# pySTEPS/pysteps

Measured on NVIDIA H100. Metric: Mpix/s advected (2048^2 frame, 12 leadtimes), higher is better.
Workload: dtype f64 (trajectories, motion field, IDW); f32 precip in/out; u8/i16/f32 OpenCV-exact LK stages

## Files before the change

### pysteps_b200/csrc/lk_track.cu

```cuda
#include "common.cuh"

namespace {

constexpr int LK_MAX_LEVELS = 8;
constexpr int LK_THREADS = 128;
constexpr int W_BITS = 14;

struct LKParams {
    const uint8_t *I, *J;
    const short2 *dI;
    size_t off[LK_MAX_LEVELS];
    int h[LK_MAX_LEVELS], w[LK_MAX_LEVELS];
    int max_level;
    int win_w, win_h, max_count;
    double eps2, min_eig_thr;
    const float *prev_pts;
    const int *npts_dev;
    int npts;
    float *next_pts;
    uint8_t *status;
};

__device__ __forceinline__ int reflect101(int i, int L) {
    if (L == 1) return 0;
    while (i < 0 || i >= L) {
        if (i < 0) i = -i;
        if (i >= L) i = 2 * L - 2 - i;
    }
    return i;
}

__device__ __forceinline__ int descale(int x, int n) { return (x + (1 << (n - 1))) >> n; }

__device__ __forceinline__ int div_small(int i, float inv_d) { return __float2int_rd(((float)i + 0.5f) * inv_d); }

__device__ __forceinline__ void make_weights(float a, float b, int &w00, int &w01, int &w10, int &w11) {
    w00 = __float2int_rn((1.f - a) * (1.f - b) * (float)(1 << W_BITS));
    w01 = __float2int_rn(a * (1.f - b) * (float)(1 << W_BITS));
    w10 = __float2int_rn((1.f - a) * b * (float)(1 << W_BITS));
    w11 = (1 << W_BITS) - w00 - w01 - w10;
}

__global__ void __launch_bounds__(LK_THREADS) lk_track_kernel(const LKParams p) {
    extern __shared__ __align__(16) unsigned char smem_raw[];
    const int npts = p.npts_dev ? min(*p.npts_dev, p.npts) : p.npts;
    const int pt = blockIdx.x;
    if (pt >= npts) return;
    const int tid = threadIdx.x;
    const int ww = p.win_w, wh = p.win_h, npx = ww * wh;
    const int simd_w = (ww / 8) * 8;
    const int nchunk = simd_w / 8, ntail = ww - simd_w;
    short *Iw = (short *)smem_raw;
    short *Dx = Iw + npx;
    short *Dy = Dx + npx;
    const int npair = wh * nchunk * 4, ntl = wh * ntail;
    float *PX = (float *)(Dy + npx + (npx & 1));
    float *PY = PX + npair;
    float *TXp = PY + npair;
    float *TYp = TXp + ntl;
    float *red = TYp + ntl;
    __shared__ float s_b[2];

    const float inv_ww = 1.0f / (float)ww, inv_nchunk = nchunk > 0 ? 1.0f / (float)nchunk : 0.f,
                inv_ntail = ntail > 0 ? 1.0f / (float)ntail : 0.f;
    const float half_x = (ww - 1) * 0.5f, half_y = (wh - 1) * 0.5f;
    const float FLT_SCALE = 1.f / (float)(1 << 20);
    const int ct = tid - 32 * (blockIdx.x & (LK_THREADS / 32 - 1));
    float nx_out = 0.f, ny_out = 0.f;
    bool status = true;

    for (int level = p.max_level; level >= 0; level--) {
        const uint8_t *I = p.I + p.off[level];
        const uint8_t *J = p.J + p.off[level];
        const short2 *dI = p.dI + p.off[level];
        const int h = p.h[level], w = p.w[level];
        const float inv = (float)(1. / (double)(1 << level));
        float px = p.prev_pts[2 * pt] * inv, py = p.prev_pts[2 * pt + 1] * inv;
        float nx, ny;
        if (level == p.max_level) { nx = px; ny = py; }
        else { nx = nx_out * 2.f; ny = ny_out * 2.f; }
        nx_out = nx; ny_out = ny;
        px -= half_x; py -= half_y;
        const int ix = __float2int_rd(px), iy = __float2int_rd(py);
        if (ix < -ww || ix >= w || iy < -wh || iy >= h) {
            if (level == 0) status = false;
            continue;
        }
        int w00, w01, w10, w11;
        make_weights(px - (float)ix, py - (float)iy, w00, w01, w10, w11);

        __syncthreads();
        const bool inI = ix >= 0 && iy >= 0 && ix + ww < w && iy + wh < h;
        for (int i = tid; i < npx; i += LK_THREADS) {
            const int y = div_small(i, inv_ww), x = i - y * ww;
            const int yy = iy + y, xx = ix + x;
            int v00, v01, v10, v11;
            short2 d00 = make_short2(0, 0), d01 = d00, d10 = d00, d11 = d00;
            if (inI) {
                const uint8_t *q0 = I + (size_t)yy * w + xx;
                v00 = q0[0]; v01 = q0[1]; v10 = q0[w]; v11 = q0[w + 1];
                const short2 *g0 = dI + (size_t)yy * w + xx;
                d00 = g0[0]; d01 = g0[1]; d10 = g0[w]; d11 = g0[w + 1];
            } else {
                const int r0 = reflect101(yy, h), r1 = reflect101(yy + 1, h);
                const int c0 = reflect101(xx, w), c1 = reflect101(xx + 1, w);
                v00 = I[(size_t)r0 * w + c0]; v01 = I[(size_t)r0 * w + c1];
                v10 = I[(size_t)r1 * w + c0]; v11 = I[(size_t)r1 * w + c1];
                const bool y0in = yy >= 0 && yy < h, y1in = yy + 1 >= 0 && yy + 1 < h;
                const bool x0in = xx >= 0 && xx < w, x1in = xx + 1 >= 0 && xx + 1 < w;
                if (y0in && x0in) d00 = dI[(size_t)yy * w + xx];
                if (y0in && x1in) d01 = dI[(size_t)yy * w + xx + 1];
                if (y1in && x0in) d10 = dI[(size_t)(yy + 1) * w + xx];
                if (y1in && x1in) d11 = dI[(size_t)(yy + 1) * w + xx + 1];
            }
            Iw[i] = (short)descale(v00 * w00 + v01 * w01 + v10 * w10 + v11 * w11, W_BITS - 5);
            Dx[i] = (short)descale(d00.x * w00 + d01.x * w01 + d10.x * w10 + d11.x * w11, W_BITS);
            Dy[i] = (short)descale(d00.y * w00 + d01.y * w01 + d10.y * w10 + d11.y * w11, W_BITS);
        }
        __syncthreads();

        if (ct >= 0 && ct < 15) {
            const int acc = ct < 12 ? ct >> 2 : ct - 12;
            const short *pa = acc == 2 ? Dy : Dx, *pb = acc == 0 ? Dx : Dy;
            float q = 0.f;
            if (ct < 12) {
                const int l = ct & 3;
                for (int y = 0; y < wh; y++) {
                    const short *ra = pa + y * ww, *rb = pb + y * ww;
#pragma unroll 4
                    for (int x = l; x < simd_w; x += 4) q = __fmul_rn((float)ra[x], (float)rb[x]) + q;
                }
            } else {
                for (int y = 0; y < wh; y++)
                    for (int x = simd_w; x < ww; x++) q += (float)((int)pa[y * ww + x] * (int)pb[y * ww + x]);
            }
            red[ct] = q;
        }
        __syncthreads();
        float A[3];
#pragma unroll
        for (int a = 0; a < 3; a++) {
            const float s = (red[4 * a + 0] + red[4 * a + 2]) + (red[4 * a + 1] + red[4 * a + 3]);
            A[a] = (red[12 + a] + s) * FLT_SCALE;
        }
        const float A11 = A[0], A12 = A[1], A22 = A[2];
        float D = A11 * A22 - A12 * A12;
        const float minEig = (A22 + A11 - sqrtf((A11 - A22) * (A11 - A22) + 4.f * A12 * A12)) /
                             (float)(2 * ww * wh);
        if ((double)minEig < p.min_eig_thr || D < 1.1920928955078125e-07f) {
            if (level == 0) status = false;
            continue;
        }
        D = 1.f / D;
        nx -= half_x; ny -= half_y;
        float pdx = 0.f, pdy = 0.f;
        for (int j = 0; j < p.max_count; j++) {
            const int jx = __float2int_rd(nx), jy = __float2int_rd(ny);
            if (jx < -ww || jx >= w || jy < -wh || jy >= h) {
                if (level == 0) status = false;
                break;
            }
            make_weights(nx - (float)jx, ny - (float)jy, w00, w01, w10, w11);
            __syncthreads();
            const bool inJ = jx >= 0 && jy >= 0 && jx + ww < w && jy + wh < h;
            auto mismatch = [&](int y, int x) -> int {
                int v00, v01, v10, v11;
                if (inJ) {
                    const uint8_t *q0 = J + (size_t)(jy + y) * w + (jx + x);
                    v00 = q0[0]; v01 = q0[1]; v10 = q0[w]; v11 = q0[w + 1];
                } else {
                    const int r0 = reflect101(jy + y, h), r1 = reflect101(jy + y + 1, h);
                    const int c0 = reflect101(jx + x, w), c1 = reflect101(jx + x + 1, w);
                    v00 = J[(size_t)r0 * w + c0]; v01 = J[(size_t)r0 * w + c1];
                    v10 = J[(size_t)r1 * w + c0]; v11 = J[(size_t)r1 * w + c1];
                }
                const int jv = descale(v00 * w00 + v01 * w01 + v10 * w10 + v11 * w11, W_BITS - 5);
                return jv - (int)Iw[y * ww + x];
            };
            for (int i = tid; i < npair; i += LK_THREADS) {
                const int q = i & 3, y = div_small(i >> 2, inv_nchunk), c = (i >> 2) - y * nchunk;
                const int x0 = 8 * c + q, i0 = y * ww + x0;
                const int d0 = mismatch(y, x0), d1 = mismatch(y, x0 + 4);
                PX[i] = (float)(d0 * (int)Dx[i0] + d1 * (int)Dx[i0 + 4]);
                PY[i] = (float)(d0 * (int)Dy[i0] + d1 * (int)Dy[i0 + 4]);
            }
            for (int i = tid; i < ntl; i += LK_THREADS) {
                const int y = div_small(i, inv_ntail), x = simd_w + (i - y * ntail);
                const int d0 = mismatch(y, x);
                TXp[i] = (float)(d0 * (int)Dx[y * ww + x]);
                TYp[i] = (float)(d0 * (int)Dy[y * ww + x]);
            }
            __syncthreads();
            if (ct >= 0 && ct < 10) {
                float q = 0.f;
                if (ct < 8) {
                    const int pair = (ct >> 2) * 2 + ((ct & 3) >> 1);
                    const float *P = (ct & 1) ? PY : PX;
                    const int nsteps = wh * nchunk;
#pragma unroll 8
                    for (int s = 0; s < nsteps; s++) q += P[4 * s + pair];
                } else {
                    const float *P = (ct == 9) ? TYp : TXp;
#pragma unroll 4
                    for (int s = 0; s < ntl; s++) q += P[s];
                }
                red[ct] = q;
            }
            __syncthreads();
            if (ct == 0) {
                const float X0 = red[0] + red[4], Y0 = red[1] + red[5];
                const float X1 = red[2] + red[6], Y1 = red[3] + red[7];
                s_b[0] = (red[8] + ((X0 + 0.f) + (X1 + 0.f))) * FLT_SCALE;
                s_b[1] = (red[9] + ((Y0 + 0.f) + (Y1 + 0.f))) * FLT_SCALE;
            }
            __syncthreads();
            const float b1 = s_b[0], b2 = s_b[1];
            const float ddx = (A12 * b2 - A22 * b1) * D;
            const float ddy = (A12 * b1 - A11 * b2) * D;
            nx += ddx; ny += ddy;
            nx_out = nx + half_x; ny_out = ny + half_y;
            if ((double)ddx * (double)ddx + (double)ddy * (double)ddy <= p.eps2) break;
            if (j > 0 && fabs((double)(ddx + pdx)) < 0.01 && fabs((double)(ddy + pdy)) < 0.01) {
                nx_out -= ddx * 0.5f; ny_out -= ddy * 0.5f;
                break;
            }
            pdx = ddx; pdy = ddy;
        }
        if (status && level == 0) {
            const int fx = __float2int_rd(nx_out - half_x), fy = __float2int_rd(ny_out - half_y);
            if (fx < -ww || fx >= w || fy < -wh || fy >= h) status = false;
        }
    }
    if (tid == 0) {
        p.next_pts[2 * pt] = nx_out;
        p.next_pts[2 * pt + 1] = ny_out;
        p.status[pt] = status ? 1 : 0;
    }
}

__global__ void __launch_bounds__(1024)
compact_tracks_kernel(const float *__restrict__ p0, const float *__restrict__ p1,
                      const uint8_t *__restrict__ st, const int *__restrict__ npts_dev, int npts_cap,
                      double *__restrict__ pool_xy, double *__restrict__ pool_uv, int *__restrict__ pool_count,
                      int pool_cap) {
    __shared__ int warp_tot[32];
    __shared__ int s_base;
    const int npts = npts_dev ? min(*npts_dev, npts_cap) : npts_cap;
    const int tid = threadIdx.x, lane = tid & 31, wid = tid >> 5;
    if (tid == 0) s_base = *pool_count;
    __syncthreads();
    for (int start = 0; start < npts; start += blockDim.x) {
        const int i = start + tid;
        const bool keep = i < npts && st[i] == 1;
        const unsigned bal = __ballot_sync(0xffffffffu, keep);
        if (lane == 0) warp_tot[wid] = __popc(bal);
        __syncthreads();
        int before = 0, total = 0;
        for (int k = 0; k < (int)(blockDim.x >> 5); k++) {
            if (k < wid) before += warp_tot[k];
            total += warp_tot[k];
        }
        if (keep) {
            const int o = s_base + before + __popc(bal & ((1u << lane) - 1u));
            if (o < pool_cap) {
                const float x0 = p0[2 * i], y0 = p0[2 * i + 1];
                pool_xy[2 * o] = (double)x0;
                pool_xy[2 * o + 1] = (double)y0;
                pool_uv[2 * o] = (double)(p1[2 * i] - x0);
                pool_uv[2 * o + 1] = (double)(p1[2 * i + 1] - y0);
            }
        }
        __syncthreads();
        if (tid == 0) s_base = min(s_base + total, pool_cap);
        __syncthreads();
    }
    if (tid == 0) *pool_count = s_base;
}

}

extern "C" int b200_lk_pyramid_layout(int h, int w, int win_w, int win_h, int max_level,
                                      int *levels_out, int64_t *offsets , int *hs, int *ws,
                                      int64_t *total_pixels) {
    B200_REQUIRE(h >= 1 && w >= 1 && win_w >= 1 && win_h >= 1 && max_level >= 0, "bad arguments");
    if (max_level > LK_MAX_LEVELS - 1) max_level = LK_MAX_LEVELS - 1;
    int lv = 0;
    int64_t off = 0;
    int ch = h, cw = w;
    for (int level = 0;; level++) {
        if (offsets) offsets[level] = off;
        if (hs) hs[level] = ch;
        if (ws) ws[level] = cw;
        off += (int64_t)ch * cw;
        lv = level;
        if (level == max_level) break;
        const int nh = (ch + 1) / 2, nw = (cw + 1) / 2;
        if (nw <= win_w || nh <= win_h) break;
        ch = nh; cw = nw;
    }
    if (levels_out) *levels_out = lv;
    if (total_pixels) *total_pixels = off;
    return 0;
}

extern "C" int b200_pyr_down_u8(const uint8_t *src, int h, int w, uint8_t *dst, void *stream);
extern "C" int b200_scharr_i16(const uint8_t *src, int h, int w, int16_t *dst, void *stream);

extern "C" int b200_lk_build_pyramid(const uint8_t *img, int h, int w, int win_w, int win_h,
                                     int max_level, uint8_t *pyr, int16_t *deriv, void *stream) {
    B200_REQUIRE(pyr && (img || deriv), "bad arguments");
    int lv, hs[LK_MAX_LEVELS], ws[LK_MAX_LEVELS];
    int64_t off[LK_MAX_LEVELS], total;
    int rc = b200_lk_pyramid_layout(h, w, win_w, win_h, max_level, &lv, off, hs, ws, &total);
    if (rc) return rc;
    cudaStream_t s = (cudaStream_t)stream;
    if (img) {
        B200_CUDA(cudaMemcpyAsync(pyr, img, (size_t)h * w, cudaMemcpyDeviceToDevice, s));
        for (int l = 1; l <= lv; l++) {
            rc = b200_pyr_down_u8(pyr + off[l - 1], hs[l - 1], ws[l - 1], pyr + off[l], stream);
            if (rc) return rc;
        }
    }
    if (deriv)
        for (int l = 0; l <= lv; l++) {
            rc = b200_scharr_i16(pyr + off[l], hs[l], ws[l], deriv + 2 * off[l], stream);
            if (rc) return rc;
        }
    return 0;
}

extern "C" int b200_lk_track(const uint8_t *pyrI, const uint8_t *pyrJ, const int16_t *derivI, int h,
                             int w, int win_w, int win_h, int max_level, int max_count, double epsilon,
                             double min_eig_thr, const float *prev_pts, int npts, const int *npts_dev,
                             float *next_pts, uint8_t *status, void *stream) {
    B200_REQUIRE(pyrI && pyrJ && derivI && prev_pts && next_pts && status, "bad arguments");
    B200_REQUIRE(win_w >= 1 && win_h >= 1 && win_w * win_h <= 64 * 64, "window must be 1..64x64 pixels");
    if (npts <= 0) return 0;
    LKParams p;
    memset(&p, 0, sizeof(p));
    int lv;
    int64_t off[LK_MAX_LEVELS], total;
    int rc = b200_lk_pyramid_layout(h, w, win_w, win_h, max_level, &lv, off, p.h, p.w, &total);
    if (rc) return rc;
    for (int l = 0; l <= lv; l++) p.off[l] = (size_t)off[l];
    p.I = pyrI; p.J = pyrJ; p.dI = (const short2 *)derivI;
    p.max_level = lv;
    p.win_w = win_w; p.win_h = win_h;
    p.max_count = max_count;
    p.eps2 = epsilon * epsilon;
    p.min_eig_thr = min_eig_thr;
    p.prev_pts = prev_pts;
    p.npts = npts; p.npts_dev = npts_dev;
    p.next_pts = next_pts; p.status = status;
    const int npx = win_w * win_h;
    const int nchunk = win_w / 8, ntail = win_w - nchunk * 8;
    const size_t smem = sizeof(short) * (3 * (size_t)npx + (npx & 1)) +
                        sizeof(float) * (2 * (size_t)win_h * nchunk * 4 + 2 * (size_t)win_h * ntail + 16);
    B200_CUDA(cudaFuncSetAttribute(lk_track_kernel, cudaFuncAttributeMaxDynamicSharedMemorySize, (int)smem));
    lk_track_kernel<<<npts, LK_THREADS, smem, (cudaStream_t)stream>>>(p);
    B200_LAUNCH_CHECK();
    return 0;
}

extern "C" int b200_lk_compact_tracks(const float *p0, const float *p1, const uint8_t *status,
                                      const int *npts_dev, int npts_cap, double *pool_xy,
                                      double *pool_uv, int *pool_count, int pool_cap, void *stream) {
    B200_REQUIRE(p0 && p1 && status && pool_xy && pool_uv && pool_count && npts_cap >= 0 && pool_cap >= 0,
                 "bad arguments");
    if (npts_cap == 0) return 0;
    compact_tracks_kernel<<<1, 1024, 0, (cudaStream_t)stream>>>(p0, p1, status, npts_dev, npts_cap, pool_xy,
                                                               pool_uv, pool_count, pool_cap);
    B200_LAUNCH_CHECK();
    return 0;
}
```

### pysteps_b200/csrc/knn.cu

```cuda
#include "common.cuh"
#include "knn_body.cuh"
#include "knn_device.cuh"

namespace {

constexpr unsigned FULL = 0xffffffffu;

struct BuildSmem {
    double kx[kdp::NMAX], ky[kdp::NMAX];
    int idx[kdp::NMAX];
    unsigned short posA[kdp::NMAX], posB[kdp::NMAX];
    int queue[2][kdp::QCAP];
    int qn[2];
    int nnodes;
};

__device__ __forceinline__ void swap3(BuildSmem &s, int p, int q) {
    const double x = s.kx[p], y = s.ky[p];
    const int i = s.idx[p];
    s.kx[p] = s.kx[q]; s.ky[p] = s.ky[q]; s.idx[p] = s.idx[q];
    s.kx[q] = x; s.ky[q] = y; s.idx[q] = i;
}

template <int MODE>
__device__ int warp_pair_partition(BuildSmem &s, const double *K, int lo, int hi, double piv, int lane) {
    const unsigned lt = (1u << lane) - 1u;
    int cntA = 0, cntB = 0;
    for (int c = lo; c < hi; c += 32) {
        const int p = c + lane;
        const bool a = p < hi && !(K[p] < piv);
        const unsigned bal = __ballot_sync(FULL, a);
        if (a) s.posA[lo + cntA + __popc(bal & lt)] = (unsigned short)p;
        cntA += __popc(bal);
    }
    for (int c = hi - 1; c >= lo; c -= 32) {
        const int p = c - lane;
        const bool b = p >= lo && (MODE == 0 ? !(piv < K[p]) : !(K[p] >= piv));
        const unsigned bal = __ballot_sync(FULL, b);
        if (b) s.posB[lo + cntB + __popc(bal & lt)] = (unsigned short)p;
        cntB += __popc(bal);
    }
    __syncwarp();
    const int npair = min(cntA, cntB);
    int j = 0;
    for (int c = 0; c < npair; c += 32) {
        const int i = c + lane;
        const bool ok = i < npair && s.posA[lo + i] < s.posB[lo + i];
        const unsigned bal = __ballot_sync(FULL, ok);
        if (ok) swap3(s, s.posA[lo + i], s.posB[lo + i]);
        j += __popc(bal);
        if (bal != FULL) break;
    }
    __syncwarp();
    if (MODE == 1) return hi - cntA;
    const int fa = j < cntA ? (int)s.posA[lo + j] : hi, fb = j > 0 ? (int)s.posB[lo + j - 1] : hi;
    return min(fa, fb);
}

__device__ void warp_nth_element(BuildSmem &s, int d, int first, int nth, int last, int lane) {
    const double *K = d ? s.ky : s.kx;
    kd::Tri tri;
    tri.kx = s.kx; tri.ky = s.ky; tri.idx = s.idx;
    int depth = 0;
    for (int m = last - first; m > 1; m >>= 1) depth++;
    depth *= 2;
    while (last - first > 3) {
        if (depth == 0) {
            if (lane == 0) {
                kd::tri_heap_select(tri, first, nth + 1, last, d);
                kd::tri_swap(tri, first, nth);
            }
            __syncwarp();
            return;
        }
        depth--;
        const int mid = first + (last - first) / 2;
        if (lane == 0) swap3(s, first, kd::tri_median_pick(K, first, mid, last));
        __syncwarp();
        const int cut = warp_pair_partition<0>(s, K, first + 1, last, K[first], lane);
        if (cut <= nth) first = cut; else last = cut;
    }
    if (lane == 0) kd::tri_insertion_sort(tri, first, last, d);
    __syncwarp();
}

__device__ __forceinline__ void write_leaf(kd::Node *nodes, int id, int start, int end) {
    kd::Node nd;
    nd.split_dim = -1; nd.less = -1; nd.greater = -1; nd.start = start; nd.end = end; nd.split = 0.0;
    nodes[id] = nd;
}

__global__ void __launch_bounds__(32 * kdp::WARPS)
kd_build_kernel(const double *__restrict__ xy, const int *__restrict__ n_dev, int n_cap, kdp::TreeBuf tb) {
    extern __shared__ __align__(16) unsigned char smem_raw[];
    BuildSmem &s = *reinterpret_cast<BuildSmem *>(smem_raw);
    const int n = n_dev ? min(*n_dev, n_cap) : n_cap;
    const int tid = threadIdx.x, lane = tid & 31, wid = tid >> 5;
    for (int i = tid; i < n; i += blockDim.x) {
        s.kx[i] = xy[2 * (size_t)i];
        s.ky[i] = xy[2 * (size_t)i + 1];
        s.idx[i] = i;
    }
    if (tid == 0) {
        s.nnodes = 1;
        s.qn[0] = n > kd::LEAFSIZE ? 1 : 0;
        s.qn[1] = 0;
        s.queue[0][0] = 0;
        write_leaf(tb.nodes, 0, 0, n);
    }
    __syncthreads();
    if (wid == 0) {
        double mx0 = n ? s.kx[0] : 0.0, mn0 = mx0, mx1 = n ? s.ky[0] : 0.0, mn1 = mx1;
        for (int i = lane; i < n; i += 32) {
            mx0 = fmax(mx0, s.kx[i]); mn0 = fmin(mn0, s.kx[i]);
            mx1 = fmax(mx1, s.ky[i]); mn1 = fmin(mn1, s.ky[i]);
        }
        for (int o = 16; o > 0; o >>= 1) {
            mx0 = fmax(mx0, __shfl_xor_sync(FULL, mx0, o)); mn0 = fmin(mn0, __shfl_xor_sync(FULL, mn0, o));
            mx1 = fmax(mx1, __shfl_xor_sync(FULL, mx1, o)); mn1 = fmin(mn1, __shfl_xor_sync(FULL, mn1, o));
        }
        if (lane == 0) { tb.bounds[0] = mx0; tb.bounds[1] = mx1; tb.bounds[2] = mn0; tb.bounds[3] = mn1; }
    }
    int cur = 0;
    for (;;) {
        const int cnt = s.qn[cur];
        if (cnt == 0) break;
        for (int w = wid; w < cnt; w += kdp::WARPS) {
            const int me = s.queue[cur][w];
            const int start = tb.nodes[me].start, end = tb.nodes[me].end;
            double mx0 = s.kx[start], mn0 = mx0, mx1 = s.ky[start], mn1 = mx1;
            for (int i = start + lane; i < end; i += 32) {
                mx0 = fmax(mx0, s.kx[i]); mn0 = fmin(mn0, s.kx[i]);
                mx1 = fmax(mx1, s.ky[i]); mn1 = fmin(mn1, s.ky[i]);
            }
            for (int o = 16; o > 0; o >>= 1) {
                mx0 = fmax(mx0, __shfl_xor_sync(FULL, mx0, o)); mn0 = fmin(mn0, __shfl_xor_sync(FULL, mn0, o));
                mx1 = fmax(mx1, __shfl_xor_sync(FULL, mx1, o)); mn1 = fmin(mn1, __shfl_xor_sync(FULL, mn1, o));
            }
            int d = 0;
            double size = 0.0;
            if (mx0 - mn0 > size) { d = 0; size = mx0 - mn0; }
            if (mx1 - mn1 > size) { d = 1; size = mx1 - mn1; }
            if ((d ? mx1 : mx0) == (d ? mn1 : mn0)) continue;
            const double *K = d ? s.ky : s.kx;
            const int nth = start + (end - start) / 2;
            warp_nth_element(s, d, start, nth, end, lane);
            double split = K[nth];
            int p = warp_pair_partition<1>(s, K, start, end, split, lane);
            if (p == start) {
                split = nextafter(split, (double)INFINITY);
                p = warp_pair_partition<1>(s, K, start, end, split, lane);
            }
            if (lane == 0) {
                const int lo = atomicAdd(&s.nnodes, 2), hi = lo + 1;
                write_leaf(tb.nodes, lo, start, p);
                write_leaf(tb.nodes, hi, p, end);
                kd::Node nd;
                nd.split_dim = d; nd.less = lo; nd.greater = hi; nd.start = start; nd.end = end; nd.split = split;
                tb.nodes[me] = nd;
                if (p - start > kd::LEAFSIZE) s.queue[cur ^ 1][atomicAdd(&s.qn[cur ^ 1], 1)] = lo;
                if (end - p > kd::LEAFSIZE) s.queue[cur ^ 1][atomicAdd(&s.qn[cur ^ 1], 1)] = hi;
            }
        }
        __syncthreads();
        if (tid == 0) s.qn[cur] = 0;
        cur ^= 1;
        __syncthreads();
    }
    for (int i = tid; i < n; i += blockDim.x) tb.idx[i] = s.idx[i];
    if (tid == 0) {
        tb.meta[0] = s.nnodes;
        tb.meta[1] = n;
        tb.meta[2] = 0;
    }
}

__global__ void kd_build_serial_kernel(const double *__restrict__ xy, const int *__restrict__ n_dev, int n_cap,
                                       kdp::TreeBuf tb) {
    if (blockIdx.x != 0 || threadIdx.x != 0) return;
    const int n = n_dev ? min(*n_dev, n_cap) : n_cap;
    int stack[128];
    kd::Tree t;
    t.data = xy;
    t.n = n;
    t.idx = tb.idx;
    t.nodes = tb.nodes;
    kd::build(t, stack);
    tb.meta[0] = t.nnodes;
    tb.meta[1] = n;
    tb.meta[2] = 0;
    for (int c = 0; c < 2; c++) {
        tb.bounds[c] = t.maxes[c];
        tb.bounds[2 + c] = t.mins[c];
    }
}

constexpr int QW = 4;

struct WarpScratch {
    kd::NodeInfo q[kdp::QHEAP];
    kd::Item nb[kdp::NBSMEM];
    double w[kdp::NBSMEM];
    int inds[kdp::NBSMEM];
};

template <class T>
__device__ __forceinline__ void wheap_push(T *h, int &n, const T &it, int lane) {
    int i = n++;
    while (i > 0 && kd::prio(it) < kd::prio(h[(i - 1) / 2])) {
        if (lane == 0) h[i] = h[(i - 1) / 2];
        i = (i - 1) / 2;
    }
    if (lane == 0) h[i] = it;
    __syncwarp();
}

template <class T>
__device__ __forceinline__ void wheap_remove(T *h, int &n, int lane) {
    const T it = h[n - 1];
    n--;
    int i = 0, j = 1, k = 2;
    while ((j < n && kd::prio(it) > kd::prio(h[j])) || (k < n && kd::prio(it) > kd::prio(h[k]))) {
        const int l = (k < n && kd::prio(h[j]) > kd::prio(h[k])) ? k : j;
        if (lane == 0) h[i] = h[l];
        i = l;
        j = 2 * i + 1;
        k = 2 * i + 2;
    }
    if (lane == 0 && n > 0) h[i] = it;
    __syncwarp();
}

__device__ void warp_query(const kd::Tree &t, const kdp::TreeBuf &tb, double x0, double x1, int kmax,
                           WarpScratch &ws, bool want_dist, int lane) {
    kd::NodeInfo *q = ws.q;
    kd::Item *nb = ws.nb;
    int qcap = kdp::QHEAP;
    const double x[2] = {x0, x1};
    int nbn = 0, qn = 0;
    kd::NodeInfo cur;
    cur.node = 0;
    cur.min_distance = 0.0;
    for (int c = 0; c < 2; c++) {
        double s = x[c] - t.maxes[c];
        const double s2 = t.mins[c] - x[c];
        if (s2 > s) s = s2;
        if (s < 0.0) s = 0.0;
        cur.side[c] = s * s;
        cur.min_distance += cur.side[c];
    }
    double dub = (double)INFINITY;
    for (;;) {
        const kd::Node node = t.nodes[cur.node];
        if (node.split_dim == -1) {
            for (int base = node.start; base < node.end; base += 32) {
                const int i = base + lane;
                const bool valid = i < node.end;
                int pi = 0;
                double d = (double)INFINITY;
                if (valid) {
                    pi = t.idx[i];
                    const double dx = t.data[2 * (size_t)pi] - x[0], dy = t.data[2 * (size_t)pi + 1] - x[1];
                    d = 0.0;
                    d += dx * dx;
                    d += dy * dy;
                }
                unsigned m = __ballot_sync(FULL, valid && d < dub);
                while (m) {
                    const int l = __ffs(m) - 1;
                    m &= m - 1;
                    const double dl = __shfl_sync(FULL, d, l);
                    const int pl = __shfl_sync(FULL, pi, l);
                    if (dl < dub) {
                        if (nbn == kmax) wheap_remove(nb, nbn, lane);
                        kd::Item it;
                        it.priority = -dl;
                        it.payload = pl;
                        wheap_push(nb, nbn, it, lane);
                        if (nbn == kmax) dub = -nb[0].priority;
                    }
                }
            }
            if (qn == 0) break;
            cur = q[0];
            wheap_remove(q, qn, lane);
        } else {
            if (cur.min_distance > dub) break;
            const int sd = node.split_dim;
            kd::NodeInfo far = cur;
            double s;
            if (x[sd] < node.split) {
                cur.node = node.less;
                far.node = node.greater;
                s = node.split - x[sd];
            } else {
                cur.node = node.greater;
                far.node = node.less;
                s = x[sd] - node.split;
            }
            s = s * s;
            far.min_distance += s - far.side[sd];
            far.side[sd] = s;
            if (cur.min_distance > far.min_distance) {
                const kd::NodeInfo tmp = cur;
                cur = far;
                far = tmp;
            }
            if (far.min_distance <= dub) {
                if (qn == qcap) {
                    const int need = tb.meta[0];
                    int off = 0;
                    if (lane == 0) off = atomicAdd(&tb.meta[2], need);
                    off = __shfl_sync(FULL, off, 0);
                    if (qcap >= need || off + need > kdp::ARENA) __trap();
                    kd::NodeInfo *big = tb.arena + off;
                    for (int e = lane; e < qn; e += 32) big[e] = q[e];
                    __syncwarp();
                    q = big;
                    qcap = need;
                }
                wheap_push(q, qn, far, lane);
            }
        }
    }
    const int found = nbn;
    for (int i = found - 1; i >= 0; i--) {
        const kd::Item top = nb[0];
        if (lane == 0) {
            ws.inds[i] = top.payload;
            if (want_dist) ws.w[i] = sqrt(-top.priority);
        }
        wheap_remove(nb, nbn, lane);
    }
    if (lane == 0)
        for (int i = found; i < kmax; i++) {
            ws.inds[i] = t.n;
            if (want_dist) ws.w[i] = (double)INFINITY;
        }
    __syncwarp();
}

struct OutlierParams {
    const double *xy, *uv;
    int k;
    double thr;
    kdp::TreeBuf tb;
    int *inds;
    kd::Item *nb;
    kd::NodeInfo *q;
    uint8_t *out;
};

__global__ void __launch_bounds__(32 * QW)
outliers_warp_kernel(const __grid_constant__ OutlierParams p) {
    __shared__ WarpScratch scratch[QW];
    const int n = p.tb.meta[1];
    const int lane = threadIdx.x & 31, wid = threadIdx.x >> 5;
    const int v = blockIdx.x * QW + wid;
    if (v >= n) return;
    if (n < 2) {
        if (lane == 0) p.out[v] = 0;
        return;
    }
    const int kk = min(p.k + 1, n);
    const kd::Tree t = kdp::tree_of(p.tb, p.xy);
    WarpScratch &ws = scratch[wid];
    warp_query(t, p.tb, p.xy[2 * (size_t)v], p.xy[2 * (size_t)v + 1], kk, ws, false, lane);
    if (lane == 0) p.out[v] = kd::mahalanobis_outlier(p.uv, v, ws.inds, kk - 1, p.thr) ? 1 : 0;
}

__global__ void __launch_bounds__(kdp::QTHREADS)
outliers_kernel(const __grid_constant__ OutlierParams p) {
    const int n = p.tb.meta[1];
    const int tid = blockIdx.x * blockDim.x + threadIdx.x;
    if (tid >= n) return;
    if (n < 2) {
        p.out[tid] = 0;
        return;
    }
    const int kk = min(p.k + 1, n);
    const kd::Tree t = kdp::tree_of(p.tb, p.xy);
    int *inds = p.inds + (size_t)tid * (p.k + 1);
    kd::Strided<kd::Item> nb{p.nb + (size_t)tid * (p.k + 1), 1};
    kd::Strided<kd::NodeInfo> q{p.q + (size_t)tid * kdp::QHEAP, 1};
    kdp::ArenaGrow grow(p.tb);
    kd::query(t, p.xy[2 * (size_t)tid], p.xy[2 * (size_t)tid + 1], kk, inds, nb, q, kdp::QHEAP, grow);
    p.out[tid] = kd::mahalanobis_outlier(p.uv, tid, inds, kk - 1, p.thr) ? 1 : 0;
}

struct IdwFixParams {
    const double *xy, *vals, *xgrid, *ygrid;
    int nvar, k, nx, ny;
    double power, offset, mean_res;
    kdp::TreeBuf tb;
    const int *list;
    const int *list_count;
    int *inds;
    double *w;
    kd::Item *nb;
    kd::NodeInfo *q;
    double *out;
    double2 *twin;
};

__global__ void __launch_bounds__(32 * QW)
idw_fix_warp_kernel(const __grid_constant__ IdwFixParams p) {
    __shared__ WarpScratch scratch[QW];
    const int n = p.tb.meta[1];
    const int k = min(p.k, n);
    const int lane = threadIdx.x & 31, wid = threadIdx.x >> 5;
    const size_t warp = (size_t)blockIdx.x * QW + wid, nwarps = (size_t)gridDim.x * QW;
    const size_t N = (size_t)p.ny * p.nx;
    const size_t count = p.list_count ? (size_t)min(*p.list_count, (int)min(N, (size_t)0x7fffffff)) : N;
    if (k < 1) return;
    const kd::Tree t = kdp::tree_of(p.tb, p.xy);
// ... 157 lines not shown
```

### pysteps_b200/csrc/knn_device.cuh

```cuda
#pragma once
#include <algorithm>

#include "common.cuh"
#include "knn_body.cuh"

namespace kdp {

constexpr int NMAX = 4096;
constexpr int WARPS = 8;
constexpr int QCAP = 512;
constexpr int QHEAP = 64;
constexpr int QTHREADS = 32;
constexpr int NBSMEM = 32;
constexpr int ARENA = 1 << 17;

struct TreeBuf {
    int *idx;
    kd::Node *nodes;
    int *meta;
    double *bounds;
    kd::NodeInfo *arena;
};

struct TreeScratch {
    b200::Scratch idx, nodes, meta, bounds, arena;
    TreeBuf tb;
};

#if defined(__CUDACC__)
__device__ __forceinline__ kd::Tree tree_of(const TreeBuf &tb, const double *xy) {
    kd::Tree t;
    t.data = xy;
    t.n = tb.meta[1];
    t.idx = tb.idx;
    t.nodes = tb.nodes;
    t.nnodes = tb.meta[0];
    for (int c = 0; c < 2; c++) {
        t.maxes[c] = tb.bounds[c];
        t.mins[c] = tb.bounds[2 + c];
    }
    return t;
}

struct ArenaGrow {
    const TreeBuf &tb;
    __device__ explicit ArenaGrow(const TreeBuf &t) : tb(t) {}
    __device__ bool operator()(kd::Strided<kd::NodeInfo> &q, int &qcap, int qn) const {
        const int need = tb.meta[0];
        if (qcap >= need) return false;
        const int off = atomicAdd(&tb.meta[2], need);
        if (off + need > ARENA) __trap();
        kd::NodeInfo *big = tb.arena + off;
        for (int i = 0; i < qn; i++) big[i] = q[i];
        q.p = big;
        q.stride = 1;
        qcap = need;
        return true;
    }
};

#endif

int tree_alloc(TreeScratch &ts, int n_cap, cudaStream_t s);
int tree_build(const double *xy, const int *n_dev, int n_cap, const TreeBuf &tb, cudaStream_t s);
int idw_fix(const double *xy, const double *vals, int nvar, int k, double power, double dist_offset,
            double mean_res, const double *xgrid, int nx, const double *ygrid, int ny, const TreeBuf &tb,
            const int *list, const int *list_count, double *out, double2 *twin, cudaStream_t s);

}
```

Before: 19300.

## Stage LK pyramid windows in shared memory with async copies and producer warps

The LK tracking kernel now copies the (win+1)^2 boxes of I, dI and J into shared memory first, using cp.async for the derivatives and word-aligned funnel-shift loads for the u8 images. Bilinear interpolation and mismatch terms then read from shared memory instead of doing scattered global loads. The gradient-matrix reduction is split so producer warps write products into a double-buffered staging area while one warp sums them, and the J box is restaged only when the integer window position changes. Reductions now read float4 vectors, one sync per iteration is dropped, and launch bounds ask for 8 blocks per SM. In exchange the shared-memory layout is more complex and the fixed summation order must still match OpenCV bit for bit.

Measured after the change: 20580, median of 6. +6.7%, better.

```diff
diff --git a/pysteps_b200/csrc/lk_track.cu b/pysteps_b200/csrc/lk_track.cu
--- a/pysteps_b200/csrc/lk_track.cu
+++ b/pysteps_b200/csrc/lk_track.cu
@@ -1,10 +1,51 @@
+#include <cuda_pipeline.h>
+
+#include <algorithm>
+
 #include "common.cuh"
 
 namespace {
 
 constexpr int LK_MAX_LEVELS = 8;
 constexpr int LK_THREADS = 128;
+constexpr int LK_PRODUCERS = LK_THREADS - 32;
+constexpr int LK_MIN_BLOCKS = 8;
+constexpr int LK_STAGE = 8;
 constexpr int W_BITS = 14;
+
+struct LKLayout {
+    int npx, nbw, nb, nbwj, nchunk, ntail, nsteps, nsteps4, ntl;
+    int srows, scs, sbuf;
+    int patch_off, box_off, jbox_off, bytes;
+};
+
+LKLayout lk_layout(int ww, int wh) {
+    LKLayout L;
+    L.npx = ww * wh;
+    L.nbw = ww + 1;
+    L.nb = (ww + 1) * (wh + 1);
+    L.nbwj = (L.nbw + 3) & ~3;
+    L.nchunk = ww / 8;
+    L.ntail = ww - 8 * L.nchunk;
+    L.nsteps = wh * L.nchunk;
+    L.nsteps4 = (L.nsteps + 3) & ~3;
+    L.ntl = wh * L.ntail;
+    L.patch_off = 64;
+    L.box_off = L.patch_off + ((6 * L.npx + 15) & ~15);
+    const int iter = 32 * L.nsteps4 + 8 * L.ntl;
+    L.jbox_off = L.box_off + iter;
+    int box = std::max(iter, 4 * L.nb) + L.nbwj * (wh + 1);
+    auto sbuf = [&](int r, int &cs) {
+        cs = (r * 2 * L.nchunk + 3) & ~3;
+        return (12 * cs + 3 * r * L.ntail + 3) & ~3;
+    };
+    L.srows = wh;
+    while (L.srows > 1 && 8 * sbuf(L.srows, L.scs) > box) L.srows--;
+    L.sbuf = sbuf(L.srows, L.scs);
+    box = std::max(box, 8 * L.sbuf);
+    L.bytes = L.box_off + ((box + 15) & ~15);
+    return L;
+}
 
 struct LKParams {
     const uint8_t *I, *J;
@@ -19,6 +60,7 @@
     int npts;
     float *next_pts;
     uint8_t *status;
+    LKLayout L;
 };
 
 __device__ __forceinline__ int reflect101(int i, int L) {
@@ -34,6 +76,17 @@
 
 __device__ __forceinline__ int div_small(int i, float inv_d) { return __float2int_rd(((float)i + 0.5f) * inv_d); }
 
+__device__ __forceinline__ void ld_pair(const short *p, bool aligned, int &lo, int &hi) {
+    if (aligned) {
+        const int v = *(const int *)p;
+        lo = (int)(short)v;
+        hi = v >> 16;
+    } else {
+        lo = p[0];
+        hi = p[1];
+    }
+}
+
 __device__ __forceinline__ void make_weights(float a, float b, int &w00, int &w01, int &w10, int &w11) {
     w00 = __float2int_rn((1.f - a) * (1.f - b) * (float)(1 << W_BITS));
     w01 = __float2int_rn(a * (1.f - b) * (float)(1 << W_BITS));
@@ -41,31 +94,92 @@
     w11 = (1 << W_BITS) - w00 - w01 - w10;
 }
 
-__global__ void __launch_bounds__(LK_THREADS) lk_track_kernel(const LKParams p) {
+__device__ __forceinline__ void stage_u8(const uint8_t *__restrict__ img, int h, int w, int ox, int oy, int nbw,
+                                         int nbh, float inv_nbw, uint8_t *__restrict__ dst, int dst_stride) {
+    const uint8_t *org = img + max(oy, 0) * w + max(ox, 0);
+    if (ox >= 0 && oy >= 0 && ox + nbw + 7 <= w && oy + nbh <= h &&
+        ((uintptr_t)org & ~(uintptr_t)3) >= (uintptr_t)img) {
+        const int nwr = dst_stride >> 2, nwords = nwr * nbh;
+        const float inv_nwr = 1.0f / (float)nwr;
+        for (int e0 = threadIdx.x; e0 < nwords; e0 += LK_STAGE * LK_THREADS) {
+            uint32_t lo[LK_STAGE], hi[LK_STAGE];
+#pragma unroll
+            for (int u = 0; u < LK_STAGE; u++) {
+                const int e = min(e0 + u * LK_THREADS, nwords - 1), r = div_small(e, inv_nwr);
+                const uint32_t *a = (const uint32_t *)((uintptr_t)(org + r * w + 4 * (e - r * nwr)) & ~(uintptr_t)3);
+                lo[u] = __ldg(a);
+                hi[u] = __ldg(a + 1);
+            }
+#pragma unroll
+            for (int u = 0; u < LK_STAGE; u++) {
+                const int e = e0 + u * LK_THREADS, r = div_small(e, inv_nwr), m = e - r * nwr;
+                const int sh = 8 * (int)((uintptr_t)(org + r * w + 4 * m) & 3);
+                if (e < nwords) ((uint32_t *)dst)[e] = __funnelshift_r(lo[u], hi[u], sh);
+            }
+        }
+        return;
+    }
+    const int nb = nbw * nbh;
+    for (int i0 = threadIdx.x; i0 < nb; i0 += LK_STAGE * LK_THREADS) {
+        uint8_t v[LK_STAGE];
+#pragma unroll
+        for (int u = 0; u < LK_STAGE; u++) {
+            const int i = min(i0 + u * LK_THREADS, nb - 1);
+            const int r = div_small(i, inv_nbw);
+            v[u] = img[reflect101(oy + r, h) * w + reflect101(ox + (i - r * nbw), w)];
+        }
+#pragma unroll
+        for (int u = 0; u < LK_STAGE; u++) {
+            const int i = i0 + u * LK_THREADS, r = div_small(i, inv_nbw);
+            if (i < nb) dst[r * dst_stride + (i - r * nbw)] = v[u];
+        }
+    }
+}
+
+__device__ __forceinline__ void stage_deriv_async(const short2 *__restrict__ der, int h, int w, int ox, int oy,
+                                                  int nbw, int nbh, float inv_nbw, short2 *__restrict__ dst) {
+    const int nb = nbw * nbh;
+    for (int i = threadIdx.x; i < nb; i += LK_THREADS) {
+        const int r = div_small(i, inv_nbw), y = oy + r, x = ox + (i - r * nbw);
+        const bool in = y >= 0 && y < h && x >= 0 && x < w;
+        __pipeline_memcpy_async(dst + i, der + (in ? y * w + x : 0), sizeof(short2), in ? 0 : sizeof(short2));
+    }
+    __pipeline_commit();
+}
+
+__global__ void __launch_bounds__(LK_THREADS, LK_MIN_BLOCKS) lk_track_kernel(const LKParams p) {
     extern __shared__ __align__(16) unsigned char smem_raw[];
     const int npts = p.npts_dev ? min(*p.npts_dev, p.npts) : p.npts;
     const int pt = blockIdx.x;
     if (pt >= npts) return;
     const int tid = threadIdx.x;
-    const int ww = p.win_w, wh = p.win_h, npx = ww * wh;
-    const int simd_w = (ww / 8) * 8;
-    const int nchunk = simd_w / 8, ntail = ww - simd_w;
-    short *Iw = (short *)smem_raw;
+    const int ww = p.win_w, wh = p.win_h;
+    const LKLayout &L = p.L;
+    const int npx = L.npx, nbw = L.nbw, nbwj = L.nbwj, nchunk = L.nchunk, ntail = L.ntail, ntl = L.ntl;
+    const int simd_w = 8 * nchunk;
+    float *red = (float *)smem_raw;
+    short *Iw = (short *)(smem_raw + L.patch_off);
     short *Dx = Iw + npx;
     short *Dy = Dx + npx;
-    const int npair = wh * nchunk * 4, ntl = wh * ntail;
-    float *PX = (float *)(Dy + npx + (npx & 1));
-    float *PY = PX + npair;
-    float *TXp = PY + npair;
+    short2 *dIb = (short2 *)(smem_raw + L.box_off);
+    uint8_t *Ib = (uint8_t *)(dIb + L.nb);
+    float *PX = (float *)(smem_raw + L.box_off);
+    float *PY = PX + 4 * L.nsteps4;
+    float *TXp = PY + 4 * L.nsteps4;
     float *TYp = TXp + ntl;
-    float *red = TYp + ntl;
-    __shared__ float s_b[2];
-
-    const float inv_ww = 1.0f / (float)ww, inv_nchunk = nchunk > 0 ? 1.0f / (float)nchunk : 0.f,
+    uint8_t *Jb = smem_raw + L.jbox_off;
+
+    const float inv_ww = 1.0f / (float)ww, inv_nbw = 1.0f / (float)nbw,
+                inv_nchunk = nchunk > 0 ? 1.0f / (float)nchunk : 0.f,
                 inv_ntail = ntail > 0 ? 1.0f / (float)ntail : 0.f;
     const float half_x = (ww - 1) * 0.5f, half_y = (wh - 1) * 0.5f;
+    const bool even = (ww & 1) == 0;
     const float FLT_SCALE = 1.f / (float)(1 << 20);
-    const int ct = tid - 32 * (blockIdx.x & (LK_THREADS / 32 - 1));
+    const int cw = blockIdx.x & (LK_THREADS / 32 - 1);
+    const int ct = tid - 32 * cw;
+    const bool producer = (tid >> 5) != cw;
+    const int ptid = tid - ((tid >> 5) > cw ? 32 : 0);
+    const int ct2 = tid - 32 * ((cw + 1) & (LK_THREADS / 32 - 1));
     float nx_out = 0.f, ny_out = 0.f;
     bool status = true;
 
@@ -90,53 +204,68 @@
         make_weights(px - (float)ix, py - (float)iy, w00, w01, w10, w11);
 
         __syncthreads();
-        const bool inI = ix >= 0 && iy >= 0 && ix + ww < w && iy + wh < h;
+        stage_deriv_async(dI, h, w, ix, iy, nbw, wh + 1, inv_nbw, dIb);
+        stage_u8(I, h, w, ix, iy, nbw, wh + 1, inv_nbw, Ib, nbwj);
+        __pipeline_wait_prior(0);
+        __syncthreads();
         for (int i = tid; i < npx; i += LK_THREADS) {
-            const int y = div_small(i, inv_ww), x = i - y * ww;
-            const int yy = iy + y, xx = ix + x;
-            int v00, v01, v10, v11;
-            short2 d00 = make_short2(0, 0), d01 = d00, d10 = d00, d11 = d00;
-            if (inI) {
-                const uint8_t *q0 = I + (size_t)yy * w + xx;
-                v00 = q0[0]; v01 = q0[1]; v10 = q0[w]; v11 = q0[w + 1];
-                const short2 *g0 = dI + (size_t)yy * w + xx;
-                d00 = g0[0]; d01 = g0[1]; d10 = g0[w]; d11 = g0[w + 1];
-            } else {
-                const int r0 = reflect101(yy, h), r1 = reflect101(yy + 1, h);
-                const int c0 = reflect101(xx, w), c1 = reflect101(xx + 1, w);
-                v00 = I[(size_t)r0 * w + c0]; v01 = I[(size_t)r0 * w + c1];
-                v10 = I[(size_t)r1 * w + c0]; v11 = I[(size_t)r1 * w + c1];
-                const bool y0in = yy >= 0 && yy < h, y1in = yy + 1 >= 0 && yy + 1 < h;
-                const bool x0in = xx >= 0 && xx < w, x1in = xx + 1 >= 0 && xx + 1 < w;
-                if (y0in && x0in) d00 = dI[(size_t)yy * w + xx];
-                if (y0in && x1in) d01 = dI[(size_t)yy * w + xx + 1];
-                if (y1in && x0in) d10 = dI[(size_t)(yy + 1) * w + xx];
-                if (y1in && x1in) d11 = dI[(size_t)(yy + 1) * w + xx + 1];
-            }
-            Iw[i] = (short)descale(v00 * w00 + v01 * w01 + v10 * w10 + v11 * w11, W_BITS - 5);
+            const int y = div_small(i, inv_ww), x = i - y * ww, b = y * nbw + x, bi = y * nbwj + x;
+            Iw[i] = (short)descale(Ib[bi] * w00 + Ib[bi + 1] * w01 + Ib[bi + nbwj] * w10 + Ib[bi + nbwj + 1] * w11,
+                                   W_BITS - 5);
+            const short2 d00 = dIb[b], d01 = dIb[b + 1], d10 = dIb[b + nbw], d11 = dIb[b + nbw + 1];
             Dx[i] = (short)descale(d00.x * w00 + d01.x * w01 + d10.x * w10 + d11.x * w11, W_BITS);
             Dy[i] = (short)descale(d00.y * w00 + d01.y * w01 + d10.y * w10 + d11.y * w11, W_BITS);
         }
         __syncthreads();
 
-        if (ct >= 0 && ct < 15) {
-            const int acc = ct < 12 ? ct >> 2 : ct - 12;
-            const short *pa = acc == 2 ? Dy : Dx, *pb = acc == 0 ? Dx : Dy;
+        {
+            const int R = L.srows, per_row = 2 * nchunk, cs = L.scs;
+            float *sbuf = (float *)(smem_raw + L.box_off);
+            const int nblk = (wh + R - 1) / R;
             float q = 0.f;
-            if (ct < 12) {
-                const int l = ct & 3;
-                for (int y = 0; y < wh; y++) {
-                    const short *ra = pa + y * ww, *rb = pb + y * ww;
+            for (int b = 0; b <= nblk; b++) {
+                if (producer && b < nblk) {
+                    float *buf = sbuf + (b & 1) * L.sbuf;
+                    const int y0 = b * R, n = min(R, wh - y0) * ww;
+                    for (int e = ptid; e < n; e += LK_PRODUCERS) {
+                        const int r = div_small(e, inv_ww), x = e - r * ww, i = (y0 + r) * ww + x;
+                        const int dx = Dx[i], dy = Dy[i];
+                        if (x < simd_w) {
+                            const float fx = (float)dx, fy = (float)dy;
+                            float *o = buf + (x & 3) * cs + r * per_row + (x >> 2);
+                            o[0] = __fmul_rn(fx, fx);
+                            o[4 * cs] = __fmul_rn(fx, fy);
+                            o[8 * cs] = __fmul_rn(fy, fy);
+                        } else {
+                            float *o = buf + 12 * cs + r * ntail + (x - simd_w);
+                            o[0] = (float)(dx * dx);
+                            o[R * ntail] = (float)(dx * dy);
+                            o[2 * R * ntail] = (float)(dy * dy);
+                        }
+                    }
+                }
+                const bool lane_chain = ct >= 0 && ct < 12, tail_chain = ct2 >= 12 && ct2 < 15;
+                if (b > 0 && (lane_chain || tail_chain)) {
+                    const float *buf = sbuf + ((b - 1) & 1) * L.sbuf;
+                    const int rows = min(R, wh - (b - 1) * R);
+                    if (lane_chain) {
+                        const float *P = buf + ct * cs;
+                        const int n = rows * per_row, n4 = n >> 2;
 #pragma unroll 4
-                    for (int x = l; x < simd_w; x += 4) q = __fmul_rn((float)ra[x], (float)rb[x]) + q;
+                        for (int k = 0; k < n4; k++) {
+                            const float4 v = reinterpret_cast<const float4 *>(P)[k];
+                            q = v.x + q; q = v.y + q; q = v.z + q; q = v.w + q;
+                        }
+                        for (int k = 4 * n4; k < n; k++) q = P[k] + q;
+                    } else {
+                        const float *P = buf + 12 * cs + (ct2 - 12) * R * ntail;
+                        for (int k = 0; k < rows * ntail; k++) q += P[k];
+                    }
+                    if (b == nblk) red[lane_chain ? ct : ct2] = q;
                 }
-            } else {
-                for (int y = 0; y < wh; y++)
-                    for (int x = simd_w; x < ww; x++) q += (float)((int)pa[y * ww + x] * (int)pb[y * ww + x]);
-            }
-            red[ct] = q;
-        }
-        __syncthreads();
+                __syncthreads();
+            }
+        }
         float A[3];
 #pragma unroll
         for (int a = 0; a < 3; a++) {
@@ -154,6 +283,8 @@
         D = 1.f / D;
         nx -= half_x; ny -= half_y;
         float pdx = 0.f, pdy = 0.f;
+        int bx = 0, by = 0;
+        bool staged = false;
         for (int j = 0; j < p.max_count; j++) {
             const int jx = __float2int_rd(nx), jy = __float2int_rd(ny);
             if (jx < -ww || jx >= w || jy < -wh || jy >= h) {
@@ -161,60 +292,74 @@
                 break;
             }
             make_weights(nx - (float)jx, ny - (float)jy, w00, w01, w10, w11);
-            __syncthreads();
-            const bool inJ = jx >= 0 && jy >= 0 && jx + ww < w && jy + wh < h;
-            auto mismatch = [&](int y, int x) -> int {
-                int v00, v01, v10, v11;
-                if (inJ) {
-                    const uint8_t *q0 = J + (size_t)(jy + y) * w + (jx + x);
-                    v00 = q0[0]; v01 = q0[1]; v10 = q0[w]; v11 = q0[w + 1];
-                } else {
-                    const int r0 = reflect101(jy + y, h), r1 = reflect101(jy + y + 1, h);
-                    const int c0 = reflect101(jx + x, w), c1 = reflect101(jx + x + 1, w);
-                    v00 = J[(size_t)r0 * w + c0]; v01 = J[(size_t)r0 * w + c1];
-                    v10 = J[(size_t)r1 * w + c0]; v11 = J[(size_t)r1 * w + c1];
+            if (!staged || jx != bx || jy != by) {
+                stage_u8(J, h, w, jx, jy, nbw, wh + 1, inv_nbw, Jb, nbwj);
+                bx = jx; by = jy; staged = true;
+                __syncthreads();
+            }
+            for (int s = tid; s < L.nsteps; s += LK_THREADS) {
+                const int y = div_small(s, inv_nchunk), x0 = 8 * (s - y * nchunk), i0 = y * ww + x0;
+                const uint8_t *r0 = Jb + y * nbwj + x0, *r1 = r0 + nbwj;
+                const uint32_t a03 = *(const uint32_t *)r0, a47 = *(const uint32_t *)(r0 + 4);
+                const uint32_t b03 = *(const uint32_t *)r1, b47 = *(const uint32_t *)(r1 + 4);
+                const int a8 = r0[8], b8 = r1[8];
+                auto px = [&](uint32_t lo, uint32_t hi, int last, int u) -> int {
+                    return u < 4 ? (int)((lo >> (8 * u)) & 255u) : u < 8 ? (int)((hi >> (8 * (u - 4))) & 255u) : last;
+                };
+                int d[8];
+#pragma unroll
+                for (int u = 0; u < 8; u += 2) {
+                    int i_lo, i_hi;
+                    ld_pair(Iw + i0 + u, even, i_lo, i_hi);
+                    d[u] = descale(px(a03, a47, a8, u) * w00 + px(a03, a47, a8, u + 1) * w01 +
+                                   px(b03, b47, b8, u) * w10 + px(b03, b47, b8, u + 1) * w11, W_BITS - 5) - i_lo;
+                    d[u + 1] = descale(px(a03, a47, a8, u + 1) * w00 + px(a03, a47, a8, u + 2) * w01 +
+                                       px(b03, b47, b8, u + 1) * w10 + px(b03, b47, b8, u + 2) * w11, W_BITS - 5) - i_hi;
                 }
-                const int jv = descale(v00 * w00 + v01 * w01 + v10 * w10 + v11 * w11, W_BITS - 5);
-                return jv - (int)Iw[y * ww + x];
-            };
-            for (int i = tid; i < npair; i += LK_THREADS) {
-                const int q = i & 3, y = div_small(i >> 2, inv_nchunk), c = (i >> 2) - y * nchunk;
-                const int x0 = 8 * c + q, i0 = y * ww + x0;
-                const int d0 = mismatch(y, x0), d1 = mismatch(y, x0 + 4);
-                PX[i] = (float)(d0 * (int)Dx[i0] + d1 * (int)Dx[i0 + 4]);
-                PY[i] = (float)(d0 * (int)Dy[i0] + d1 * (int)Dy[i0 + 4]);
-            }
-            for (int i = tid; i < ntl; i += LK_THREADS) {
-                const int y = div_small(i, inv_ntail), x = simd_w + (i - y * ntail);
-                const int d0 = mismatch(y, x);
+#pragma unroll
+                for (int k = 0; k < 2; k++) {
+                    const short *G = k ? Dy : Dx;
+                    float *P = k ? PY : PX;
+                    int g[8];
+#pragma unroll
+                    for (int u = 0; u < 8; u += 2) ld_pair(G + i0 + u, even, g[u], g[u + 1]);
+#pragma unroll
+                    for (int c = 0; c < 4; c++) P[c * L.nsteps4 + s] = (float)(d[c] * g[c] + d[c + 4] * g[c + 4]);
+                }
+            }
+            for (int i = (tid + LK_THREADS - L.nsteps % LK_THREADS) % LK_THREADS; i < ntl; i += LK_THREADS) {
+                const int y = div_small(i, inv_ntail), x = simd_w + (i - y * ntail), b = y * nbwj + x;
+                const int d0 = descale(Jb[b] * w00 + Jb[b + 1] * w01 + Jb[b + nbwj] * w10 + Jb[b + nbwj + 1] * w11,
+                                       W_BITS - 5) - (int)Iw[y * ww + x];
                 TXp[i] = (float)(d0 * (int)Dx[y * ww + x]);
                 TYp[i] = (float)(d0 * (int)Dy[y * ww + x]);
             }
             __syncthreads();
-            if (ct >= 0 && ct < 10) {
+            const bool lane_chain = ct >= 0 && ct < 8;
+            if (lane_chain || ct2 == 8 || ct2 == 9) {
                 float q = 0.f;
-                if (ct < 8) {
+                if (lane_chain) {
                     const int pair = (ct >> 2) * 2 + ((ct & 3) >> 1);
-                    const float *P = (ct & 1) ? PY : PX;
-                    const int nsteps = wh * nchunk;
-#pragma unroll 8
-                    for (int s = 0; s < nsteps; s++) q += P[4 * s + pair];
+                    const float *P = ((ct & 1) ? PY : PX) + pair * L.nsteps4;
+                    const int n4 = L.nsteps >> 2;
+#pragma unroll 4
+                    for (int s = 0; s < n4; s++) {
+                        const float4 v = reinterpret_cast<const float4 *>(P)[s];
+                        q += v.x; q += v.y; q += v.z; q += v.w;
+                    }
+                    for (int s = 4 * n4; s < L.nsteps; s++) q += P[s];
                 } else {
-                    const float *P = (ct == 9) ? TYp : TXp;
+                    const float *P = (ct2 == 9) ? TYp : TXp;
 #pragma unroll 4
                     for (int s = 0; s < ntl; s++) q += P[s];
                 }
-                red[ct] = q;
+                red[lane_chain ? ct : ct2] = q;
             }
             __syncthreads();
-            if (ct == 0) {
-                const float X0 = red[0] + red[4], Y0 = red[1] + red[5];
-                const float X1 = red[2] + red[6], Y1 = red[3] + red[7];
-                s_b[0] = (red[8] + ((X0 + 0.f) + (X1 + 0.f))) * FLT_SCALE;
-                s_b[1] = (red[9] + ((Y0 + 0.f) + (Y1 + 0.f))) * FLT_SCALE;
-            }
-            __syncthreads();
-            const float b1 = s_b[0], b2 = s_b[1];
+            const float X0 = red[0] + red[4], Y0 = red[1] + red[5];
+            const float X1 = red[2] + red[6], Y1 = red[3] + red[7];
+            const float b1 = (red[8] + ((X0 + 0.f) + (X1 + 0.f))) * FLT_SCALE;
+            const float b2 = (red[9] + ((Y0 + 0.f) + (Y1 + 0.f))) * FLT_SCALE;
             const float ddx = (A12 * b2 - A22 * b1) * D;
             const float ddy = (A12 * b1 - A11 * b2) * D;
             nx += ddx; ny += ddy;
@@ -352,11 +497,10 @@
     p.prev_pts = prev_pts;
     p.npts = npts; p.npts_dev = npts_dev;
     p.next_pts = next_pts; p.status = status;
-    const int npx = win_w * win_h;
-    const int nchunk = win_w / 8, ntail = win_w - nchunk * 8;
-    const size_t smem = sizeof(short) * (3 * (size_t)npx + (npx & 1)) +
-                        sizeof(float) * (2 * (size_t)win_h * nchunk * 4 + 2 * (size_t)win_h * ntail + 16);
-    B200_CUDA(cudaFuncSetAttribute(lk_track_kernel, cudaFuncAttributeMaxDynamicSharedMemorySize, (int)smem));
+    p.L = lk_layout(win_w, win_h);
+    B200_REQUIRE((int64_t)h * w <= INT32_MAX, "frame must have fewer than 2^31 pixels");
+    const int smem = p.L.bytes;
+    B200_CUDA(cudaFuncSetAttribute(lk_track_kernel, cudaFuncAttributeMaxDynamicSharedMemorySize, smem));
     lk_track_kernel<<<npts, LK_THREADS, smem, (cudaStream_t)stream>>>(p);
     B200_LAUNCH_CHECK();
     return 0;
```

## Hold kNN neighbor heap in warp registers and widen kd-tree build

Applied to the files above, without the earlier changes.

The warp-cooperative k-nearest-neighbor query now keeps its bounded max-heap distributed across lane registers. Push and remove work through ballots and shuffles along the sift path, replacing the shared-memory heap that only lane 0 updated. The kd-tree build keeps each queued node's start/end range in shared memory instead of re-reading it from global node records. It also raises the build block from 8 to 32 warps, and indexes the split dimension with selects instead of dynamic array indexing. These changes target latency in the tree build and query used for IDW interpolation. The cost is more shuffle traffic, a heap capacity tied to 32 lanes, and extra shared memory.

Result: no change. 20080 before, 20180 after (median of 6 runs) (+0.5%).

```diff
diff --git a/pysteps_b200/csrc/knn.cu b/pysteps_b200/csrc/knn.cu
--- a/pysteps_b200/csrc/knn.cu
+++ b/pysteps_b200/csrc/knn.cu
@@ -11,6 +11,7 @@
     int idx[kdp::NMAX];
     unsigned short posA[kdp::NMAX], posB[kdp::NMAX];
     int queue[2][kdp::QCAP];
+    int qs[2][kdp::QCAP], qe[2][kdp::QCAP];
     int qn[2];
     int nnodes;
 };
@@ -106,6 +107,8 @@
         s.qn[0] = n > kd::LEAFSIZE ? 1 : 0;
         s.qn[1] = 0;
         s.queue[0][0] = 0;
+        s.qs[0][0] = 0;
+        s.qe[0][0] = n;
         write_leaf(tb.nodes, 0, 0, n);
     }
     __syncthreads();
@@ -127,7 +130,7 @@
         if (cnt == 0) break;
         for (int w = wid; w < cnt; w += kdp::WARPS) {
             const int me = s.queue[cur][w];
-            const int start = tb.nodes[me].start, end = tb.nodes[me].end;
+            const int start = s.qs[cur][w], end = s.qe[cur][w];
             double mx0 = s.kx[start], mn0 = mx0, mx1 = s.ky[start], mn1 = mx1;
             for (int i = start + lane; i < end; i += 32) {
                 mx0 = fmax(mx0, s.kx[i]); mn0 = fmin(mn0, s.kx[i]);
@@ -158,8 +161,15 @@
                 kd::Node nd;
                 nd.split_dim = d; nd.less = lo; nd.greater = hi; nd.start = start; nd.end = end; nd.split = split;
                 tb.nodes[me] = nd;
-                if (p - start > kd::LEAFSIZE) s.queue[cur ^ 1][atomicAdd(&s.qn[cur ^ 1], 1)] = lo;
-                if (end - p > kd::LEAFSIZE) s.queue[cur ^ 1][atomicAdd(&s.qn[cur ^ 1], 1)] = hi;
+                const int nx = cur ^ 1;
+                if (p - start > kd::LEAFSIZE) {
+                    const int e = atomicAdd(&s.qn[nx], 1);
+                    s.queue[nx][e] = lo; s.qs[nx][e] = start; s.qe[nx][e] = p;
+                }
+                if (end - p > kd::LEAFSIZE) {
+                    const int e = atomicAdd(&s.qn[nx], 1);
+                    s.queue[nx][e] = hi; s.qs[nx][e] = p; s.qe[nx][e] = end;
+                }
             }
         }
         __syncthreads();
@@ -199,9 +209,55 @@
 
 struct WarpScratch {
     kd::NodeInfo q[kdp::QHEAP];
-    kd::Item nb[kdp::NBSMEM];
     double w[kdp::NBSMEM];
     int inds[kdp::NBSMEM];
+};
+
+struct RegHeap {
+    double pr;
+    int pay;
+    int n;
+
+    __device__ __forceinline__ void push(double ipr, int ipay, int lane) {
+        const int slot = n++;
+        const int sh = __clz(lane + 1) - __clz(slot + 1);
+        const bool path = sh >= 0 && ((slot + 1) >> sh) == lane + 1;
+        const bool down = path && lane != slot && ipr < pr;
+        const unsigned D = __ballot_sync(FULL, down);
+        const int par = (lane - 1) >> 1;
+        const double ppr = __shfl_sync(FULL, pr, par & 31);
+        const int ppay = __shfl_sync(FULL, pay, par & 31);
+        if (path) {
+            if (lane > 0 && ((D >> par) & 1u)) { pr = ppr; pay = ppay; }
+            else if (lane == slot || down) { pr = ipr; pay = ipay; }
+        }
+    }
+
+    __device__ __forceinline__ void remove(int lane) {
+        const double ipr = __shfl_sync(FULL, pr, (n - 1) & 31);
+        const int ipay = __shfl_sync(FULL, pay, (n - 1) & 31);
+        n--;
+        const int j = 2 * lane + 1, k = j + 1;
+        const double pj = __shfl_sync(FULL, pr, j & 31), pk = __shfl_sync(FULL, pr, k & 31);
+        const bool right = k < n && pj > pk;
+        const int l = right ? k : j;
+        const int cpay = __shfl_sync(FULL, pay, l & 31);
+        const unsigned R = __ballot_sync(FULL, right);
+        unsigned P = 1u;
+        for (int a = 0; 2 * a + 1 < n;) {
+            a = 2 * a + 1 + (int)((R >> a) & 1u);
+            P |= 1u << a;
+        }
+        const bool path = (P >> lane) & 1u;
+        const bool up = path && lane > 0 && ipr > pr;
+        const unsigned U = __ballot_sync(FULL, up);
+        if (path && n > 0) {
+            if (j < n && ((U >> l) & 1u)) { pr = right ? pk : pj; pay = cpay; }
+            else if (lane == 0 || up) { pr = ipr; pay = ipay; }
+        }
+    }
+
+    __device__ __forceinline__ double top_priority() const { return __shfl_sync(FULL, pr, 0); }
 };
 
 template <class T>
@@ -234,10 +290,13 @@
 __device__ void warp_query(const kd::Tree &t, const kdp::TreeBuf &tb, double x0, double x1, int kmax,
                            WarpScratch &ws, bool want_dist, int lane) {
     kd::NodeInfo *q = ws.q;
-    kd::Item *nb = ws.nb;
+    RegHeap nb;
+    nb.pr = 0.0;
+    nb.pay = 0;
+    nb.n = 0;
     int qcap = kdp::QHEAP;
     const double x[2] = {x0, x1};
-    int nbn = 0, qn = 0;
+    int qn = 0;
     kd::NodeInfo cur;
     cur.node = 0;
     cur.min_distance = 0.0;
@@ -272,12 +331,9 @@
                     const double dl = __shfl_sync(FULL, d, l);
                     const int pl = __shfl_sync(FULL, pi, l);
                     if (dl < dub) {
-                        if (nbn == kmax) wheap_remove(nb, nbn, lane);
-                        kd::Item it;
-                        it.priority = -dl;
-                        it.payload = pl;
-                        wheap_push(nb, nbn, it, lane);
-                        if (nbn == kmax) dub = -nb[0].priority;
+                        if (nb.n == kmax) nb.remove(lane);
+                        nb.push(-dl, pl, lane);
+                        if (nb.n == kmax) dub = -nb.top_priority();
                     }
                 }
             }
@@ -288,19 +344,20 @@
             if (cur.min_distance > dub) break;
             const int sd = node.split_dim;
             kd::NodeInfo far = cur;
+            const double xs = sd ? x1 : x0;
             double s;
-            if (x[sd] < node.split) {
+            if (xs < node.split) {
                 cur.node = node.less;
                 far.node = node.greater;
-                s = node.split - x[sd];
+                s = node.split - xs;
             } else {
                 cur.node = node.greater;
                 far.node = node.less;
-                s = x[sd] - node.split;
+                s = xs - node.split;
             }
             s = s * s;
-            far.min_distance += s - far.side[sd];
-            far.side[sd] = s;
+            far.min_distance += s - (sd ? far.side[1] : far.side[0]);
+            if (sd) far.side[1] = s; else far.side[0] = s;
             if (cur.min_distance > far.min_distance) {
                 const kd::NodeInfo tmp = cur;
                 cur = far;
@@ -323,14 +380,13 @@
             }
         }
     }
-    const int found = nbn;
+    const int found = nb.n;
     for (int i = found - 1; i >= 0; i--) {
-        const kd::Item top = nb[0];
         if (lane == 0) {
-            ws.inds[i] = top.payload;
-            if (want_dist) ws.w[i] = sqrt(-top.priority);
-        }
-        wheap_remove(nb, nbn, lane);
+            ws.inds[i] = nb.pay;
+            if (want_dist) ws.w[i] = sqrt(-nb.pr);
+        }
+        nb.remove(lane);
     }
     if (lane == 0)
         for (int i = found; i < kmax; i++) {
diff --git a/pysteps_b200/csrc/knn_device.cuh b/pysteps_b200/csrc/knn_device.cuh
--- a/pysteps_b200/csrc/knn_device.cuh
+++ b/pysteps_b200/csrc/knn_device.cuh
@@ -7,7 +7,7 @@
 namespace kdp {
 
 constexpr int NMAX = 4096;
-constexpr int WARPS = 8;
+constexpr int WARPS = 32;
 constexpr int QCAP = 512;
 constexpr int QHEAP = 64;
 constexpr int QTHREADS = 32;
```
